# SonghuaHu-UMD/MultiSTGraph

Hardware: AMD Instinct MI355X
Metric: forward node-steps/s (B*T*N per second), MultiATGCN.predict (higher is better)
Workload: dtype f32; 1 GPU; Baltimore 403-node, in=24h out=24h, batch=64/GPU, multi+unidirection K=5; nodes=403, per_gpu_batch=64, global_batch=64, in_steps=24, out_steps=24, parallelism=batch shards, no data-path collective (dp1), layer_wavefront_streams=True

## Files before the change

multistgraph_amd/csrc/matgcn_bwd.hip:

```cpp

namespace {

template <class V, size_t n, class Match, class Args>
int launch_chain(const V (&table)[n], Match match, const dim3& grid, int lds, hipStream_t s, const Args& a) {
  const V* v = find_variant(table, match);
  if (!v) return MATGCN_ERR_UNSUPPORTED;
  hipLaunchKernelGGL(v->fn, grid, dim3(512), lds, s, a);
  CHECK_LAUNCH();
  return MATGCN_OK;
}
constexpr int MAX_FUSED_PARTS = 4;
struct ChainResVariant { bool carry; int parts; bool bf; void (*fn)(ChainResNodeArgs); };
const ChainResVariant CHAIN_RES[] = {
    {false, 0, false, k_chain_res_node<false, true, 0>}, {false, 0, true, k_chain_res_node<false, true, 0, true>},
    {true, 0, false, k_chain_res_node<true, true, 0>},   {true, 0, true, k_chain_res_node<true, true, 0, true>},
    {true, 1, false, k_chain_res_node<true, true, 1>},   {true, 1, true, k_chain_res_node<true, true, 1, true>},
    {true, 2, false, k_chain_res_node<true, true, 2>},   {true, 2, true, k_chain_res_node<true, true, 2, true>},
    {true, 3, false, k_chain_res_node<true, true, 3>},   {true, 3, true, k_chain_res_node<true, true, 3, true>},
    {true, MAX_FUSED_PARTS, false, k_chain_res_node<true, true, MAX_FUSED_PARTS>},
    {true, MAX_FUSED_PARTS, true, k_chain_res_node<true, true, MAX_FUSED_PARTS, true>},
};
struct ChainGateVariant { int parts; bool beta, bf; void (*fn)(ChainNodeArgs); };
const ChainGateVariant CHAIN_GATE[] = {
    {0, false, false, k_chain_gate_node<0, false>}, {0, true, false, k_chain_gate_node<0, true>},
// ... 1286 lines not shown
}

}

extern "C" {

int matgcn_train_bytes(const matgcn_dims* dims, size_t* bytes) {
  if (!bytes) return MATGCN_ERR_NULL;
  Plan P;
  RETURN_IF(make_plan(dims, &P));
  TrainPlan R;
  RETURN_IF(make_train_plan(P, &R));
  *bytes = (size_t)((g_train_precision == 2 && !P.gcnOff ? R.floatsBf16 : R.floats) + (g_deterministic ? R.detFloats : 0)) *
           sizeof(float);
  return MATGCN_OK;
}

static int forward_train_impl(const matgcn_dims* dims, const matgcn_params* params, const void* prepared, const float* X,
                              const matgcn_series* src, const float* h0, const float* drop_mask, float* out,
                              void* workspace, size_t workspace_bytes, void* train, size_t train_bytes, void* stream) {
  if (!prepared || (!X && !src) || !out || !train) return MATGCN_ERR_NULL;
  if (src) RETURN_IF(check_series(dims, src->series, src->series_steps, src->label_start, src->rel_steps));
  Ctx c;
  RETURN_IF(make_ctx(&c, dims, params, prepared, workspace, workspace_bytes, stream, false));
  if (!params->weight_tsg || !params->end_conv_bias) return MATGCN_ERR_NULL;
  for (int h = 0; h < dims->n_heads; ++h) if (!params->weight_ts[h]) return MATGCN_ERR_NULL;
  RETURN_IF(check_layer_params(dims, params));
  const Plan& P = c.P;
  RETURN_IF(make_train_plan(P, &c.R));
  if (train_bytes < (size_t)c.R.floats * sizeof(float)) return MATGCN_ERR_SMALL_BUFFER;
  c.train = (float*)train;
  const int mode = g_train_precision;
  if (mode == 2 && !P.gcnOff && (workspace_bytes < (size_t)P.workspaceFloatsBf16 * sizeof(float) ||
                                 train_bytes < (size_t)c.R.floatsBf16 * sizeof(float)))
    return MATGCN_ERR_SMALL_BUFFER;
  c.prec = precision_of(mode);
  note_train_mode(train, -1);
  if (P.Np != P.N) {
    const size_t rows = (size_t)(c.R.savedFloats / ((long)P.Np * H));
    hipLaunchKernelGGL(k_zero_pad_rows, dim3(blocks_for(rows * (P.Np - P.N) * H)), dim3(256), 0, c.s, c.train,
                       (int)rows, P.N, P.Np, H);
    CHECK_LAUNCH();
  }
  RETURN_IF(wavefront_ready());
  const bool side = g_wavefront_mode != 0;
  hipStream_t aux = side ? g_wf.aux : c.s;
  if (side) {
    HIP_OK(hipEventRecord(g_wf.auxFork, c.s));
    HIP_OK(hipStreamWaitEvent(aux, g_wf.auxFork, 0));
  }
  RETURN_IF(plain_operands(c, c.train, aux, mode == 2 && !P.gcnOff));
  if (side) HIP_OK(hipEventRecord(g_wf.auxDone, aux));
  float* x0p = c.ws + P.oX0p;
  if (src) RETURN_IF(fuse_padded(c, src->series, x0p, src->label_start, src->rel_steps, src->series_steps));
  else RETURN_IF(fuse_padded(c, X, x0p));
  const bool fusedDrop = drop_mask != nullptr && !P.gcnOff;
  if (fusedDrop) c.dropMask = drop_mask;
  RETURN_IF(encoder_padded(c, x0p, h0, nullptr));
  if (side) HIP_OK(hipStreamWaitEvent(c.s, g_wf.auxDone, 0));
  const float* seqTop = c.ws + P.oSeq[P.L - 1];
  if (fusedDrop) {
    seqTop = c.train + c.R.oSeqDrop;
  } else if (drop_mask) {
    const size_t ofs = (size_t)(P.T - P.headT) * P.B * P.Np * H;
    float* dropped = c.train + c.R.oSeqDrop;
    hipLaunchKernelGGL(k_apply_mask, dim3(blocks_for((size_t)P.headT * P.B * P.Np * H)), dim3(256), 0, c.s, seqTop + ofs,
                       drop_mask, dropped + ofs, P.B, P.headT, P.N, P.Np);
    CHECK_LAUNCH();
    seqTop = dropped;
  }
  RETURN_IF(head_padded(c, seqTop, out));
  note_train_mode(train, mode);
  return MATGCN_OK;
}

static int forward_train_entry(const matgcn_dims* dims, const matgcn_params* params, const void* prepared, const float* X,
                               const matgcn_series* src, const float* h0, const float* drop_mask, float* out, void* workspace,
                               size_t workspace_bytes, void* train, size_t train_bytes, void* stream) {
  JOINED(forward_train_impl(dims, params, prepared, X, src, h0, drop_mask, out, workspace, workspace_bytes, train,
                            train_bytes, stream), stream);
}

int matgcn_forward_train(const matgcn_dims* dims, const matgcn_params* params, const void* prepared, const float* X,
                         const matgcn_series* src, const float* h0, const float* drop_mask, float* out, void* workspace,
                         size_t workspace_bytes, void* train, size_t train_bytes, void* stream) {
  return on_main_stream(stream, [&](void* s) {
    return forward_train_entry(dims, params, prepared, X, src, h0, drop_mask, out, workspace, workspace_bytes, train,
                               train_bytes, s);
  });
}

static int backward_entry(const matgcn_dims* dims, const matgcn_params* params, const void* prepared, const float* X,
                          const matgcn_series* src, const float* h0, const float* drop_mask, const float* d_out,
                          const matgcn_grads* grads, float* d_h0, void* workspace, size_t workspace_bytes, void* train,
                          size_t train_bytes, void* stream) {
  if (!prepared || (!X && !src) || !d_out || !grads || !train) return MATGCN_ERR_NULL;
  if (src) RETURN_IF(check_series(dims, src->series, src->series_steps, src->label_start, src->rel_steps));
  Bwd b;
  RETURN_IF(make_ctx(&b.c, dims, params, prepared, workspace, workspace_bytes, stream));
  RETURN_IF(check_layer_params(dims, params));
  RETURN_IF(make_train_plan(b.c.P, &b.c.R));
  if (train_bytes < (size_t)b.c.R.floats * sizeof(float)) return MATGCN_ERR_SMALL_BUFFER;
  b.X = X; b.dropMask = drop_mask; b.g = grads; b.tr = (float*)train;
  b.hasH0 = h0 != nullptr; b.dH0 = d_h0; b.src = src;
  const int mode = train_mode_of(train);
  if (mode < 0) return MATGCN_ERR_BAD_ARG;
  if (mode == 2 && !b.c.P.gcnOff && train_bytes < (size_t)b.c.R.floatsBf16 * sizeof(float)) return MATGCN_ERR_SMALL_BUFFER;
  b.c.prec = precision_of(mode);
  if (g_deterministic) {
    const long base = mode == 2 && !b.c.P.gcnOff ? b.c.R.floatsBf16 : b.c.R.floats;
    if (train_bytes < (size_t)(base + b.c.R.detFloats) * sizeof(float)) return MATGCN_ERR_SMALL_BUFFER;
// ... 34 lines not shown
```

multistgraph_amd/csrc/matgcn_capi.hip:

```cpp
#include <hip/hip_runtime.h>
#include <stdint.h>
#include <stdio.h>
#include <stdlib.h>
#include <string.h>

#include "../../include/matgcn.h"
#include "matgcn_internal.h"

#include "matgcn_kernels.hip"
#include "matgcn_node16.hip"
#include "matgcn_bwd_kernels.hip"

namespace {

constexpr int H = 64;
constexpr int MAX_STEPS = 64;
constexpr int X_CHUNK = 2;

inline long rup(long v, long m) { return (v + m - 1) / m * m; }

struct Plan {
  int B, N, Np, T, L, C0, Ks, Ktot, nFirst, Mp, Kx, d, CH, NTc, od, Tc;
  int per, KtotOrig, nDenseFirst;
  int sumDense;
// ... 580 lines not shown
  const dim3 grid((unsigned)(a.nRowTiles * ((a.nColTiles * 64 + tile.cols - 1) / tile.cols)), (unsigned)a.parts);
  hipLaunchKernelGGL(v->fn, grid, dim3(256), 0, s, a);
  return launch_ok();
}

inline bool mix_flush(MixPrec prec, const MixArgs& a) { return prec != MIX_BF16 && a.nK > 64; }
inline bool mix_half_tiles(MixPrec prec, const MixArgs& a) {
  return prec == MIX_F32 && !mix_flush(prec, a) && a.nColTiles <= 16 && a.xTileStride % 4 == 0 && a.ldX >= 64;
}
inline bool mix_x3_ok(const MixArgs& a) { return a.Apl != nullptr && a.xTileStride % 2 == 0 && a.ldX % 2 == 0; }

struct MixOps { MixPrec prec; const float* St; const void* planes; };
inline MixOps mix_ops(const Ctx& c) {
  return MixOps{c.prec.mix, c.prep + c.P.oSt, c.prec.mix == MIX_BF16X3 ? c.ws + c.P.oPlanes : nullptr};
}

int launch_mix(const Plan& P, const MixOps& m, const float* X, long xTileStride, int ldX, int nColTiles,
               float* out, long sN, long sK, long sT, int Ks, int rowsM, hipStream_t s, bool stepRole = false,
               long outFloats = 0) {
  if (Ks <= 0 || rowsM <= 0) return MATGCN_OK;
  MixArgs a;
  a.St = m.St; a.ldS = P.Mp; a.X = X; a.xTileStride = xTileStride; a.ldX = ldX;
  a.Apl = m.planes; a.plStride = P.planeWords;
  a.out = out; a.sN = sN; a.sK = sK; a.sT = sT; a.outFloats = outFloats;
  a.Np = P.Np; a.N = P.N; a.Ks = Ks; a.nK = P.Np / 16; a.nColTiles = nColTiles;
  ProfScope prof(stepRole ? MATGCN_PROF_MIX : MATGCN_PROF_MIX_PRE, s);
  const MixPrec prec = m.prec;
  if (prec == MIX_BF16X3 && !mix_x3_ok(a)) return MATGCN_ERR_UNSUPPORTED;
  const MixTile tile = prec == MIX_BF16X3 ? MIX_64x128 : mix_half_tiles(prec, a) ? MIX_64x32 : MIX_64x64;
  return launch_mix_variant(tile, prec, mix_flush(prec, a), stepRole ? 1 : 0, a, rowsM, s);
}

int mix_rows(const Plan& P, const MixOps& m, const float* X, int rows, float* G, hipStream_t s, bool stepRole = false,
             long nodeStride = 0) {
  const long sN = nodeStride ? nodeStride : (long)rows * P.Ks * H;
  return launch_mix(P, m, X, (long)P.Np * H, H, rows, G, sN, H, (long)P.Ks * H, P.Ks, P.Ks * P.Np, s, stepRole,
                    (long)(P.N - 1) * sN + (long)rows * P.Ks * H);
}

int lds_opt_in(const void* kernel, int bytes) {
  HIP_OK(hipFuncSetAttribute(kernel, hipFuncAttributeMaxDynamicSharedMemorySize, bytes));
  return MATGCN_OK;
}
int node_kernels_ready(int ldsBytes) {
  int& ready = dev_current().nodeLds;
  if (ready >= ldsBytes) return MATGCN_OK;
  for (const NodeVariant& v : GATE16) RETURN_IF(lds_opt_in(reinterpret_cast<const void*>(v.fn), v.lds));
  for (const NodeVariant& v : UPDATE16) RETURN_IF(lds_opt_in(reinterpret_cast<const void*>(v.fn), v.lds));
  for (const PxVariant& v : PX16) RETURN_IF(lds_opt_in(reinterpret_cast<const void*>(v.fn), ldsBytes));
  ready = ldsBytes;
  return MATGCN_OK;
}

int fold_x0(const Ctx& c, const float* xin, int Tq, hipStream_t s) {
  const Plan& P = c.P;
  const int rows = P.B * Tq;
  const int ld = (int)rup((long)rows * P.C0, 64);
  float* X0m = c.ws + P.oX0m;
  float* MX0 = c.ws + P.oMX0;
  hipLaunchKernelGGL(k_x0_to_matrix, dim3(blocks_for((size_t)P.Np * ld)), dim3(256), 0, s, xin, X0m, rows, P.Np, P.C0,
                     ld);
  CHECK_LAUNCH();
  RETURN_IF(launch_mix(P, mix_ops(c), X0m, 64, ld, ld / 64, MX0, (long)ld, (long)P.Np * ld, 64, P.Ks, P.Ks * P.Np, s));
  hipLaunchKernelGGL(k_build_xa0, dim3(blocks_for((size_t)Tq * P.N * P.B * P.Kx)), dim3(256), 0, s, xin, MX0,
                     c.ws + P.oXA0, P.B, Tq, P.N, P.Np, P.C0, P.Ks, P.Kx, ld);
  return launch_ok();
}

inline int chunk_steps(const Plan& P, int t) {
  int nt = (t < 2) ? 1 : (t < 4 ? 2 : P.Tc);
  if (nt > P.Tc) nt = P.Tc;
  if (t + nt > P.T) nt = P.T - t;
  return nt;
}

int hoist_x(const Ctx& c, int l, const float* xin, int t0, int nt, hipStream_t s, int mixedSteps = 0) {
  const Plan& P = c.P;
  const int rows = P.B * nt;
  float* GX = (c.train ? c.train + c.R.oGX[l] : c.ws + P.oGX[l]) + (size_t)t0 * P.N * P.B * P.Ks * H;
  if (mixedSteps < nt) {
    const int r0 = mixedSteps * P.B;
    RETURN_IF(mix_rows(P, mix_ops(c), xin + (size_t)mixedSteps * P.B * P.Np * H, rows - r0,
                       GX + (size_t)r0 * P.Ks * H, s, false, mixedSteps ? (long)rows * P.Ks * H : 0));
  }
  Px16Args a;
  a.x = xin; a.g = GX; a.w = c.prep + P.oWx[l]; a.bias = c.prep + P.oBx[l];
  a.pxOut = c.ws + P.oPX[l] + (size_t)t0 * P.N * P.RB * NODE_PX_BLOCK;
  a.steps = nt; a.N = P.N; a.Np = P.Np; a.Ks = P.Ks; a.B = P.B;
  ProfScope prof(MATGCN_PROF_PX, s);
  const dim3 grid((unsigned)(rup(P.N, 8) * nt * P.RB));
  const bool bf = c.prec.node;
  if (bf) a.w = c.ws + P.oW16x[l];
  const int nrt = P.B <= 16 ? 1 : P.B <= 32 ? 2 : 4;
  const PxVariant* v = find_variant(PX16, [&](auto& e) { return e.nrt == nrt && e.bf == bf; });
  if (!v) return MATGCN_ERR_UNSUPPORTED;
  hipLaunchKernelGGL(v->fn, grid, dim3(512), P.nodeLds, s, a);
  return launch_ok();
}

bool shared_mix_slot(const Ctx& c, int l, int t, float** g, long* nodeStride) {
  const Plan& P = c.P;
  if (P.gcnOff || l + 1 >= P.L || t < 0 || t >= P.T || P.Ks <= 0) return false;
  int t0 = 0;
  while (t0 + chunk_steps(P, t0) <= t) t0 += chunk_steps(P, t0);
  const int nt = chunk_steps(P, t0);
  const size_t gStep = (size_t)P.N * P.B * P.Ks * H;
  *g = (c.train ? c.train + c.R.oGX[l + 1] : c.ws + P.oGX[l + 1]) + t0 * gStep + (size_t)(t - t0) * P.B * P.Ks * H;
  *nodeStride = (long)nt * P.B * P.Ks * H;
  return true;
}

void fill_res_args(const Ctx& c, int l, const float* xt, long xRowStride, const float* blend, float* seq_t,
                   Node16Args* a) {
  const Plan& P = c.P;
  a->xt = xt; a->xRowStride = xRowStride; a->C = P.Cl[l]; a->Cpad = P.Cpad[l];
// ... 24 lines not shown
  else a.px = c.ws + P.oPX[l] + (size_t)t * P.N * P.RB * NODE_PX_BLOCK;
  const bool save = c.train != nullptr && res != nullptr;
  const bool rows32 = (P.B <= 32 || P.N <= 256) && res != nullptr && !raw && !c.prec.node;
  const dim3 grid(node_items(P.N, P.B, rows32 ? 32 : 64));
  if (save) {
    const size_t at = (size_t)t * P.B * P.Np * H;
    a.svZ = c.train + c.R.oZ[l] + at; a.svR = c.train + c.R.oR[l] + at; a.svHC = c.train + c.R.oHC[l] + at;
    a.svZ2 = c.train + c.R.oZ2[l] + at; a.svR2 = c.train + c.R.oR2[l] + at; a.svHC2 = c.train + c.R.oHC2[l] + at;
  }
  const bool bf = c.prec.node && res != nullptr && !raw;
  if (phase == 1) {
    a.s = Hx; a.w = bf ? c.ws + P.oW16g[l] : c.prep + P.oWg[l]; a.zh = ZHx; a.r = R; a.raw = raw;
    ProfScope prof(MATGCN_PROF_GATE, s);
    return launch_node(GATE16, 0, save, rows32 ? 32 : 64, bf, zeroState, grid, s, a);
  }
  a.s = ZHx; a.w = bf ? c.ws + P.oW16u[l] : c.prep + P.oWu[l]; a.r = R; a.h = Hx; a.hout = Hx;
  ProfScope prof(MATGCN_PROF_UPDATE, s);
  if (res) {
    a.xt = res->xt; a.xRowStride = res->xRowStride; a.C = res->C; a.Cpad = res->Cpad;
    a.rg = res->rg; a.rgb = res->rgb; a.ru = res->ru; a.rub = res->rub;
    a.blend = res->blend; a.seq = res->seq; a.seqRowStride = res->seqRowStride;
    if (save && c.dropMask && l == P.L - 1 && t >= P.T - P.headT && a.seq) {
      a.dropMask = c.dropMask + (size_t)(t - (P.T - P.headT)) * P.N * H;
      a.dropRowStride = (long)P.headT * P.N * H;
      a.seqDrop = c.train + c.R.oSeqDrop + (a.seq - (c.ws + P.oSeq[l]));
    }
  }
  return launch_node(UPDATE16, res ? 1 : 0, save, rows32 ? 32 : 64, bf, zeroState, grid, s, a);
}

int cell_step(const Ctx& c, int l, int t, float* raw, bool gateOnly, const Node16Args* res, hipStream_t s) {
  RETURN_IF(cell_phase(c, l, t, 0, raw, res, s));
  RETURN_IF(cell_phase(c, l, t, 1, raw, res, s));
  if (gateOnly) return MATGCN_OK;
  RETURN_IF(cell_phase(c, l, t, 2, nullptr, res, s));
  return cell_phase(c, l, t, 3, nullptr, res, s);
}

int res_step(const Ctx& c, int l, const float* xt, long xRowStride) {
  const Plan& P = c.P;
  Node16Args a;
  memset(&a, 0, sizeof(a));
  a.s = c.ws + P.oHx[l]; a.hout = c.ws + P.oHx[l];
  a.rows = P.B; a.N = P.N; a.Np = P.Np; a.Ks = P.Ks;
  fill_res_args(c, l, xt, xRowStride, nullptr, nullptr, &a);
  ProfScope prof(MATGCN_PROF_RES, c.s);
  return launch_node(UPDATE16, 2, false, 64, false, false, dim3(node_items(P.N, P.B, 64)), c.s, a);
}

int zero_async(float* p, long floats, hipStream_t s) {
  return hipMemsetAsync(p, 0, (size_t)floats * sizeof(float), s) == hipSuccess ? MATGCN_OK : MATGCN_ERR_LAUNCH;
}

int encoder_chains(const Ctx& c, const float* x0p, const float* h0User, float* finalsUser) {
  const Plan& P = c.P;
  RETURN_IF(node_kernels_ready(P.nodeLds));
  RETURN_IF(wavefront_ready());
  Wavefront& W = g_wf;
  const bool multi = P.L > 1 && g_wavefront_mode != 0;
  const bool lazyPrep = prep_current().pending;
  const bool zeroStart = !h0User && !c.train && !P.gcnOff;
  if (lazyPrep && (!multi || c.prec.node || P.gcnOff)) RETURN_IF(prep_wait(c.s, 3));
  if (c.prec.node && !P.gcnOff) {
    if (c.wsBytes < (size_t)P.workspaceFloatsBf16 * sizeof(float)) return MATGCN_ERR_SMALL_BUFFER;
    for (int l = 0; l < P.L; ++l) {
      const size_t og = (size_t)(P.wgFloats[l] / 8), ou = (size_t)(P.wuFloats[l] / 8);
      hipLaunchKernelGGL(k_stream_to_bf16, dim3(blocks_for(og)), dim3(256), 0, c.s, c.prep + P.oWg[l],
                         reinterpret_cast<unsigned int*>(c.ws + P.oW16g[l]), og);
      CHECK_LAUNCH();
      hipLaunchKernelGGL(k_stream_to_bf16, dim3(blocks_for(ou)), dim3(256), 0, c.s, c.prep + P.oWu[l],
                         reinterpret_cast<unsigned int*>(c.ws + P.oW16u[l]), ou);
      CHECK_LAUNCH();
      if (l > 0) {
        const size_t ox = (size_t)((long)P.N * P.wxStride / 8);
        hipLaunchKernelGGL(k_stream_to_bf16, dim3(blocks_for(ox)), dim3(256), 0, c.s, c.prep + P.oWx[l],
                           reinterpret_cast<unsigned int*>(c.ws + P.oW16x[l]), ox);
        CHECK_LAUNCH();
      }
    }
  }
  if (c.prec.mix == MIX_BF16X3 && P.Ks > 0) {
    if (c.wsBytes < (size_t)P.workspaceFloatsX3 * sizeof(float)) return MATGCN_ERR_SMALL_BUFFER;
    hipLaunchKernelGGL(k_split_bf16x3, dim3(blocks_for((size_t)P.planeWords)), dim3(256), 0, c.s, c.prep + P.oSt, P.Mp, P.Np,
                       P.nKg, reinterpret_cast<uint4*>(c.ws + P.oPlanes), P.planeWords);
    CHECK_LAUNCH();
  }
  if (multi) {
    HIP_OK(hipEventRecord(W.fork, c.s));
    for (int l = 1; l < P.L; ++l) {
      HIP_OK(hipStreamWaitEvent(W.chain[l], W.fork, 0));
      HIP_OK(hipStreamWaitEvent(W.xpart[l], W.fork, 0));
      if (lazyPrep) {
        RETURN_IF(prep_wait(W.chain[l], 2));
        RETURN_IF(prep_wait(W.xpart[l], 2));
      }
    }
  }
  if (!P.gcnOff) RETURN_IF(fold_x0(c, x0p, P.T, c.s));
  const long stepRows = (long)P.B * P.Np * H;
  auto chain_stream = [&](int l) { return (l == 0 || !multi) ? c.s : W.chain[l]; };
  for (int l = 0; l < P.L; ++l) {
    hipStream_t cs = chain_stream(l);
    RETURN_IF(zero_async(c.ws + P.oZHx[l], (long)P.B * P.Np * H, cs));
    if (P.Np != P.N) {
      hipLaunchKernelGGL(k_zero_pad_rows, dim3(blocks_for((size_t)P.B * P.T * (P.Np - P.N) * H)), dim3(256), 0, cs,
                         c.ws + P.oSeq[l], P.B * P.T, P.N, P.Np, H);
      CHECK_LAUNCH();
    }
    hipLaunchKernelGGL(k_pack_rows, dim3(blocks_for((size_t)P.B * P.Np * H)), dim3(256), 0, cs,
                       h0User ? h0User + (size_t)l * P.B * P.N * H : nullptr,
                       c.ws + P.oHx[l], P.B, P.N, P.Np, H);
    CHECK_LAUNCH();
    if (c.train && h0User) {
      hipLaunchKernelGGL(k_pack_rows, dim3(blocks_for((size_t)P.B * P.Np * H)), dim3(256), 0, cs,
                         h0User + (size_t)l * P.B * P.N * H, c.train + c.R.oH0 + (size_t)l * P.B * P.Np * H, P.B, P.N,
                         P.Np, H);
      CHECK_LAUNCH();
    }
  }
  int nextChunk[MATGCN_MAX_LAYERS] = {0};
  auto enqueue_step = [&](int l, int t) -> int {
    hipStream_t cs = chain_stream(l);
    hipStream_t xs = multi ? W.xpart[l] : c.s;
    const float* below = (l == 0) ? nullptr : c.ws + P.oSeq[l - 1];
    float* seq = c.ws + P.oSeq[l];
    if (P.gcnOff) {
      if (multi && l > 0) HIP_OK(hipStreamWaitEvent(cs, W.step[l - 1][t], 0));
      Node16Args a;
      memset(&a, 0, sizeof(a));
      a.s = c.ws + P.oHx[l]; a.hout = c.ws + P.oHx[l];
      a.rows = P.B; a.N = P.N; a.Np = P.Np; a.Ks = 0;
      if (l == 0) fill_res_args(c, l, x0p + (long)t * P.Np * P.C0, (long)P.T * P.Np * P.C0, nullptr, seq + t * stepRows, &a);
      else fill_res_args(c, l, below + t * stepRows, (long)P.Np * H, nullptr, seq + t * stepRows, &a);
      {
        ProfScope prof(MATGCN_PROF_RES, cs);
        if (c.train) {
          const size_t at = (size_t)t * P.B * P.Np * H;
          a.svZ2 = c.train + c.R.oZ2[l] + at; a.svR2 = c.train + c.R.oR2[l] + at; a.svHC2 = c.train + c.R.oHC2[l] + at;
        }
        RETURN_IF(launch_node(UPDATE16, 2, c.train != nullptr, 64, false, false, dim3(node_items(P.N, P.B, 64)), cs, a));
      }
      CHECK_LAUNCH();
      if (multi && l + 1 < P.L) HIP_OK(hipEventRecord(W.step[l][t], cs));
      return MATGCN_OK;
    }
    if (l > 0 && t == nextChunk[l]) {
      const int nt = chunk_steps(P, t);
      nextChunk[l] = t + nt;
      float* slot; long stride;
      int mixedSteps = 0;
      if (shared_mix_slot(c, l - 1, t, &slot, &stride)) mixedSteps = P.T - 1 - t < nt ? P.T - 1 - t : nt;
      if (multi) {
        if (mixedSteps == nt) HIP_OK(hipStreamWaitEvent(xs, W.mixed[l - 1][t + nt], 0));
        else HIP_OK(hipStreamWaitEvent(xs, W.step[l - 1][t + nt - 1], 0));
      }
      RETURN_IF(hoist_x(c, l, below + t * stepRows, t, nt, xs, mixedSteps));
      if (multi) {
        HIP_OK(hipEventRecord(W.xdone[l][t], xs));
        HIP_OK(hipStreamWaitEvent(cs, W.xdone[l][t], 0));
      }
    }
    Node16Args res;
    if (l == 0)
      fill_res_args(c, l, x0p + (long)t * P.Np * P.C0, (long)P.T * P.Np * P.C0,
                    c.prm->weights_gru + (size_t)l * P.T + t, seq + t * stepRows, &res);
    else
      fill_res_args(c, l, below + t * stepRows, (long)P.Np * H, c.prm->weights_gru + (size_t)l * P.T + t,
                    seq + t * stepRows, &res);
    const bool zs = zeroStart && t == 0;
    if (!zs) RETURN_IF(cell_phase(c, l, t, 0, nullptr, &res, cs));
    if (multi && l + 1 < P.L) HIP_OK(hipEventRecord(W.mixed[l][t], cs));
    if (lazyPrep && multi && l == 0 && t == 0) RETURN_IF(prep_wait(cs, 1));
    RETURN_IF(cell_phase(c, l, t, 1, nullptr, &res, cs, zs));
    if (!zs) RETURN_IF(cell_phase(c, l, t, 2, nullptr, &res, cs));
    RETURN_IF(cell_phase(c, l, t, 3, nullptr, &res, cs, zs));
    if (multi && l + 1 < P.L) HIP_OK(hipEventRecord(W.step[l][t], cs));
    return MATGCN_OK;
  };
  for (int l = 0; l < P.L; ++l)
    for (int t = 0; t < P.T; ++t) RETURN_IF(enqueue_step(l, t));
  for (int l = 0; l < P.L; ++l) {
    hipStream_t cs = chain_stream(l);
    if (finalsUser) {
      hipLaunchKernelGGL(k_unpack_rows, dim3(blocks_for((size_t)P.B * P.N * H)), dim3(256), 0, cs, c.ws + P.oHx[l],
                         finalsUser + (size_t)l * P.B * P.N * H, P.B, P.N, P.Np, H);
      CHECK_LAUNCH();
    }
    if (multi && l > 0) HIP_OK(hipEventRecord(W.done[l], cs));
  }
  if (multi)
    for (int l = 1; l < P.L; ++l) HIP_OK(hipStreamWaitEvent(c.s, W.done[l], 0));
  return MATGCN_OK;
}

int encoder_padded(const Ctx& c, const float* x0p, const float* h0User, float* finalsUser) {
  const int rc = encoder_chains(c, x0p, h0User, finalsUser);
  if (rc != MATGCN_OK) join_library_streams(c.s);
  return rc;
}

int fuse_padded(const Ctx& c, const float* X, float* x0p, const int32_t* labelStart = nullptr,
                const int32_t* relSteps = nullptr, int64_t seriesSteps = 0) {
  const Plan& P = c.P;
  const matgcn_dims* D = c.D;
  RETURN_IF(zero_async(x0p, (long)P.B * P.T * P.Np * P.C0, c.s));
  FuseArgs a;
  memset(&a, 0, sizeof(a));
  a.X = X; a.x0 = x0p; a.tsg = c.prm->weight_tsg;
  a.labelStart = labelStart; a.seriesSteps = (long)seriesSteps;
  if (labelStart)
    for (int s2 = 0; s2 < D->x_steps; ++s2) a.rel[s2] = relSteps[s2];
  for (int h = 0; h < D->n_heads; ++h) { a.ts[h] = c.prm->weight_ts[h]; a.headBegin[h] = D->head_begin[h]; }
  for (int j = 0; j < P.C0 - P.od; ++j) a.extSrc[j] = D->ext_src[j];
  a.B = P.B; a.T = P.T; a.N = P.N; a.Np = P.Np; a.C0 = P.C0; a.od = P.od; a.F = D->x_feat;
  a.xSteps = D->x_steps; a.startDim = D->start_dim; a.nHeads = D->n_heads; a.nTs = D->n_ts;
  hipLaunchKernelGGL(k_fuse_heads, dim3(blocks_for((size_t)P.B * P.T * P.N)), dim3(256), 0, c.s, a);
  return launch_ok();
}

int head_padded(const Ctx& c, const float* seqp, float* out) {
  const Plan& P = c.P;
  HeadArgs a;
  a.seq = seqp + (size_t)(P.T - P.headT) * P.B * P.Np * H; a.w = c.prep + P.oHead;
  a.bias = c.prm->end_conv_bias; a.out = out;
  a.B = P.B; a.T = P.headT; a.N = P.N; a.Np = P.Np; a.CH = P.CH; a.od = P.od; a.NTc = P.NTc;
  ProfScope prof(MATGCN_PROF_HEAD, c.s);
  hipLaunchKernelGGL(k_head, dim3((unsigned)(P.B * ((P.N + 31) / 32))), dim3(256), 0, c.s, a);
  return launch_ok();
}

int make_ctx(Ctx* c, const matgcn_dims* dims, const matgcn_params* params, const void* prepared, void* workspace,
             size_t workspace_bytes, void* stream, bool joinPrepare = true) {
  if (!dims || !params || !workspace) return MATGCN_ERR_NULL;
  RETURN_IF(make_plan(dims, &c->P));
  if (workspace_bytes < (size_t)c->P.workspaceFloats * sizeof(float)) return MATGCN_ERR_SMALL_BUFFER;
  c->D = dims; c->prm = params; c->prep = (const float*)prepared; c->ws = (float*)workspace;
  c->wsBytes = workspace_bytes;
  c->s = (hipStream_t)stream;
  if (prepared && joinPrepare) RETURN_IF(prep_wait(c->s, 3));
  return MATGCN_OK;
}

int check_layer_params(const matgcn_dims* D, const matgcn_params* p) {
  if (!D->gcn_off && (!p->node_emb || !p->weights_gru)) return MATGCN_ERR_NULL;
  for (int l = 0; l < D->layers; ++l) {
    if (!p->res_gate[l].weight || !p->res_gate[l].bias || !p->res_update[l].weight || !p->res_update[l].bias)
      return MATGCN_ERR_NULL;
    if (D->gcn_off) continue;
    if (!p->gate[l].weights_pool || !p->gate[l].bias_pool || !p->update[l].weights_pool || !p->update[l].bias_pool)
      return MATGCN_ERR_NULL;
    if (D->scale_by_g && (!p->gate[l].weights_g || !p->update[l].weights_g)) return MATGCN_ERR_NULL;
    if (!p->res_gate[l].weight || !p->res_gate[l].bias || !p->res_update[l].weight || !p->res_update[l].bias)
      return MATGCN_ERR_NULL;
  }
  return MATGCN_OK;
}

int stage_single_step(const Ctx& c, int layer, const float* x, const float* h, bool xpart, float** xin_out) {
  const Plan& P = c.P;
  if (layer < 0 || layer >= P.L) return MATGCN_ERR_BAD_ARG;
  if (P.gcnOff && xpart) return MATGCN_ERR_UNSUPPORTED;
  RETURN_IF(node_kernels_ready(P.nodeLds));
  float* xin = (layer == 0) ? c.ws + P.oX0p : c.ws + P.oSeq[layer - 1];
  hipLaunchKernelGGL(k_pack_rows, dim3(blocks_for((size_t)P.B * P.Np * P.Cl[layer])), dim3(256), 0, c.s, x, xin, P.B,
                     P.N, P.Np, P.Cl[layer]);
  CHECK_LAUNCH();
  hipLaunchKernelGGL(k_pack_rows, dim3(blocks_for((size_t)P.B * P.Np * H)), dim3(256), 0, c.s, h, c.ws + P.oHx[layer],
                     P.B, P.N, P.Np, H);
  CHECK_LAUNCH();
// ... 297 lines not shown
      if (l == 0) {
        if (!fast) {
          q.baseOfs = (long)nG * 16 * O; q.kind = 1; q.iOfs = 0; q.groups = P.nGx[0];
          hipLaunchKernelGGL(k_prep_stream<1>, dim3(blocks_for((size_t)q.groups * (O / 16) * 64), nodeGroups), dim3(256), 0,
                             ws, q);
          CHECK_LAUNCH();
        }
      } else {
        q.out = prep + P.oWx[l]; q.nodeStride = P.wxStride; q.baseOfs = 0;
        q.kind = 0; q.iOfs = 0; q.groups = nG; q.OTdst = 12; q.otOfs = part == 0 ? 0 : 8;
        if (fast)
          launch_fast(q, O, ws);
        else
          hipLaunchKernelGGL(k_prep_stream<0>, dim3(blocks_for((size_t)q.groups * (O / 16) * 64), nodeGroups), dim3(256), 0,
                             ws, q);
        CHECK_LAUNCH();
        hipLaunchKernelGGL(k_prep_bias, dim3(blocks_for((size_t)P.N * O)), dim3(256), 0, ws, params->node_emb,
                           ap.bias_pool, P.d, O, P.N, prep + P.oBx[l], 192, part == 0 ? 0 : 128);
        CHECK_LAUNCH();
      }
    }
    if (lazy && l == 0) {
      HIP_OK(hipEventRecord(E.l0[0], pool[1]));
      HIP_OK(hipEventRecord(E.l0[1], pool[2]));
    }
    const int nG1 = (P.Cpad[l] + H) / 16;
    hipLaunchKernelGGL(k_prep_linear16, dim3(blocks_for((size_t)nG1 * 8 * 64)), dim3(256), 0, c.s,
                       params->res_gate[l].weight, I, 128, P.Cl[l], P.Cpad[l], nG1, prep + P.oRg[l]);
    CHECK_LAUNCH();
    hipLaunchKernelGGL(k_prep_linear16, dim3(blocks_for((size_t)nG1 * 4 * 64)), dim3(256), 0, c.s,
                       params->res_update[l].weight, I, 64, P.Cl[l], P.Cpad[l], nG1, prep + P.oRu[l]);
    CHECK_LAUNCH();
  }
  hipLaunchKernelGGL(k_prep_linear, dim3(blocks_for((size_t)(P.headT * H / 8) * P.NTc * 64)), dim3(256), 0, c.s,
                     params->end_conv_weight, P.headT * H, P.CH, 0, 0, P.headT * H, P.NTc, prep + P.oHead);
  CHECK_LAUNCH();
  if (lazy) {
    HIP_OK(hipEventRecord(E.l1[0], pool[1]));
    HIP_OK(hipEventRecord(E.l1[1], pool[2]));
    E.pending = true;
  } else if (fork) {
    HIP_OK(hipEventRecord(W.done[1], pool[1]));
    HIP_OK(hipEventRecord(W.done[2], pool[2]));
    HIP_OK(hipStreamWaitEvent(c.s, W.done[1], 0));
    HIP_OK(hipStreamWaitEvent(c.s, W.done[2], 0));
  }
  return MATGCN_OK;
}

static int forward_once(Ctx& c, const float* X, const float* series, int64_t seriesSteps, const int32_t* labelStart,
                        const int32_t* relSteps, const float* h0, float* out) {
  const Plan& P = c.P;
  float* x0p = c.ws + P.oX0p;
  if (series) RETURN_IF(fuse_padded(c, series, x0p, labelStart, relSteps, seriesSteps));
  else RETURN_IF(fuse_padded(c, X, x0p));
  RETURN_IF(encoder_padded(c, x0p, h0, nullptr));
  return head_padded(c, c.ws + P.oSeq[P.L - 1], out);
}

static int forward_entry(const matgcn_dims* dims, const matgcn_params* params, const void* prepared, const float* X,
                         const float* h0, float* out, void* workspace, size_t workspace_bytes, void* stream) {
  if (!prepared || !X || !out) return MATGCN_ERR_NULL;
  Ctx c;
  RETURN_IF(make_ctx(&c, dims, params, prepared, workspace, workspace_bytes, stream, false));
  if (!params->weight_tsg || !params->end_conv_bias) return MATGCN_ERR_NULL;
  for (int h = 0; h < dims->n_heads; ++h) if (!params->weight_ts[h]) return MATGCN_ERR_NULL;
  RETURN_IF(check_layer_params(dims, params));
  c.prec = precision_of(g_mix_precision);
  return forward_once(c, X, nullptr, 0, nullptr, nullptr, h0, out);
}

int matgcn_forward(const matgcn_dims* dims, const matgcn_params* params, const void* prepared, const float* X,
                   const float* h0, float* out, void* workspace, size_t workspace_bytes, void* stream) {
  return on_main_stream(stream, [&](void* s) {
    return forward_entry(dims, params, prepared, X, h0, out, workspace, workspace_bytes, s);
  });
}

static int check_series(const matgcn_dims* dims, const float* series, int64_t series_steps, const int32_t* label_start,
                 const int32_t* rel_steps) {
  if (!series || !label_start || !rel_steps) return MATGCN_ERR_NULL;
  if (dims->x_steps > MATGCN_MAX_XSTEPS) return MATGCN_ERR_UNSUPPORTED;
  int lo = 0;
  for (int s2 = 0; s2 < dims->x_steps; ++s2) lo = rel_steps[s2] < lo ? rel_steps[s2] : lo;
  if (series_steps < 1 || -(int64_t)lo >= series_steps) return MATGCN_ERR_BAD_ARG;
  return MATGCN_OK;
}

static int forward_series_entry(const matgcn_dims* dims, const matgcn_params* params, const void* prepared,
                                const float* series, int64_t series_steps, const int32_t* label_start,
                                const int32_t* rel_steps, const float* h0, float* out, void* workspace,
                                size_t workspace_bytes, void* stream) {
  if (!prepared || !series || !label_start || !rel_steps || !out) return MATGCN_ERR_NULL;
  Ctx c;
  RETURN_IF(make_ctx(&c, dims, params, prepared, workspace, workspace_bytes, stream, false));
  if (!params->weight_tsg || !params->end_conv_bias) return MATGCN_ERR_NULL;
  for (int h = 0; h < dims->n_heads; ++h) if (!params->weight_ts[h]) return MATGCN_ERR_NULL;
  RETURN_IF(check_layer_params(dims, params));
  RETURN_IF(check_series(dims, series, series_steps, label_start, rel_steps));
  c.prec = precision_of(g_mix_precision);
  return forward_once(c, nullptr, series, series_steps, label_start, rel_steps, h0, out);
}

int matgcn_forward_series(const matgcn_dims* dims, const matgcn_params* params, const void* prepared,
                          const float* series, int64_t series_steps, const int32_t* label_start,
                          const int32_t* rel_steps, const float* h0, float* out, void* workspace,
                          size_t workspace_bytes, void* stream) {
  return on_main_stream(stream, [&](void* s) {
    return forward_series_entry(dims, params, prepared, series, series_steps, label_start, rel_steps, h0, out, workspace,
                                workspace_bytes, s);
  });
}

int matgcn_fuse_heads(const matgcn_dims* dims, const matgcn_params* params, const float* X, float* x0,
                      void* workspace, size_t workspace_bytes, void* stream) {
  if (!X || !x0) return MATGCN_ERR_NULL;
  Ctx c;
  RETURN_IF(make_ctx(&c, dims, params, nullptr, workspace, workspace_bytes, stream));
  if (!params->weight_tsg) return MATGCN_ERR_NULL;
  for (int h = 0; h < dims->n_heads; ++h) if (!params->weight_ts[h]) return MATGCN_ERR_NULL;
  const Plan& P = c.P;
  float* x0p = c.ws + P.oX0p;
  RETURN_IF(fuse_padded(c, X, x0p));
  hipLaunchKernelGGL(k_unpack_rows, dim3(blocks_for((size_t)P.B * P.T * P.N * P.C0)), dim3(256), 0, c.s, x0p, x0,
                     P.B * P.T, P.N, P.Np, P.C0);
  return launch_ok();
}

int matgcn_agcn_gate_fwd(const matgcn_dims* dims, const matgcn_params* params, const void* prepared, int layer,
                         const float* x, const float* h, float* y, void* workspace, size_t workspace_bytes,
                         void* stream) {
  if (!prepared || !x || !h || !y) return MATGCN_ERR_NULL;
  Ctx c;
  RETURN_IF(make_ctx(&c, dims, params, prepared, workspace, workspace_bytes, stream));
  float* xin;
  RETURN_IF(stage_single_step(c, layer, x, h, true, &xin));
  return cell_step(c, layer, 0, y, true, nullptr, c.s);
}

int matgcn_atgru_cell_fwd(const matgcn_dims* dims, const matgcn_params* params, const void* prepared, int layer,
                          const float* x, const float* h, float* h_out, void* workspace, size_t workspace_bytes,
                          void* stream) {
  if (!prepared || !x || !h || !h_out) return MATGCN_ERR_NULL;
  Ctx c;
  RETURN_IF(make_ctx(&c, dims, params, prepared, workspace, workspace_bytes, stream));
  const Plan& P = c.P;
  float* xin;
  RETURN_IF(stage_single_step(c, layer, x, h, true, &xin));
  RETURN_IF(cell_step(c, layer, 0, nullptr, false, nullptr, c.s));
  hipLaunchKernelGGL(k_unpack_rows, dim3(blocks_for((size_t)P.B * P.N * H)), dim3(256), 0, c.s, c.ws + P.oHx[layer],
                     h_out, P.B, P.N, P.Np, H);
  return launch_ok();
}

int matgcn_res_cell_fwd(const matgcn_dims* dims, const matgcn_params* params, const void* prepared, int layer,
                        const float* x, const float* h, float* h_out, void* workspace, size_t workspace_bytes,
                        void* stream) {
  if (!prepared || !x || !h || !h_out) return MATGCN_ERR_NULL;
  Ctx c;
  RETURN_IF(make_ctx(&c, dims, params, prepared, workspace, workspace_bytes, stream));
  const Plan& P = c.P;
  float* xin;
  RETURN_IF(stage_single_step(c, layer, x, h, false, &xin));
  RETURN_IF(res_step(c, layer, xin, (long)P.Np * P.Cl[layer]));
  hipLaunchKernelGGL(k_unpack_rows, dim3(blocks_for((size_t)P.B * P.N * H)), dim3(256), 0, c.s, c.ws + P.oHx[layer],
                     h_out, P.B, P.N, P.Np, H);
  return launch_ok();
}

int matgcn_encoder_fwd(const matgcn_dims* dims, const matgcn_params* params, const void* prepared, const float* x0,
                       const float* h0, float* seq, float* finals, void* workspace, size_t workspace_bytes,
                       void* stream) {
  if (!prepared || !x0) return MATGCN_ERR_NULL;
  Ctx c;
  RETURN_IF(make_ctx(&c, dims, params, prepared, workspace, workspace_bytes, stream));
  RETURN_IF(check_layer_params(dims, params));
// ... 67 lines not shown
```

multistgraph_amd/csrc/matgcn_internal.h:

```cpp
#ifndef MATGCN_INTERNAL_H
#define MATGCN_INTERNAL_H
#include <stddef.h>
#include <stdint.h>

#define MATGCN_MAX_STACK 16

struct StackMap {
  int KtotOrig;
  int nKeep;
  int keepK[MATGCN_MAX_STACK];
  int nDiag;
  int diagK[MATGCN_MAX_STACK];
  int diagOrder[MATGCN_MAX_STACK];
  const float* diagSrc[MATGCN_MAX_STACK];
  int N;
};

struct StackEntries {
  int n;
  int pool[2 * MATGCN_MAX_STACK];
  int slot[2 * MATGCN_MAX_STACK];
  int diag[2 * MATGCN_MAX_STACK];
};

struct PrepStream {
  const float* E;
  const float* wpool;
  const float* bpool;
  const float* wg;
  float* out;
  long nodeStride;
  long baseOfs;
  int d, I, O, N;
  int kind;
  int iOfs, C0;
  int groups;
  int groupsX;
  int OTdst, otOfs;
  StackMap map;
};

struct FuseArgs {
  const float* X;
  const int* labelStart;
  int rel[256];
  long seriesSteps;
  float* x0;
  const float* tsg;
  const float* ts[8];
  int B, T, N, Np, C0, od, F, xSteps, startDim, nHeads, nTs;
  int headBegin[8];
  int extSrc[16];
};

struct MixArgs {
  const float* St = nullptr;
  int ldS = 0;
  const float* X = nullptr;
  long xTileStride = 0;
  int ldX = 0;
  float* out = nullptr;
  long sN = 0, sK = 0, sT = 0;
  long outFloats = 0;
  int Np = 0, N = 0, Ks = 0, nK = 0, nColTiles = 0, nRowTiles = 0;
  int parts = 1;
  long aPartStride = 0, xPartStride = 0, outPartStride = 0;
  const void* Apl = nullptr;
  long plStride = 0;
};

struct HeadArgs {
  const float* seq;
  const float* w;
  const float* bias;
  float* out;
  int B, T, N, Np, CH, od, NTc;
};

#endif
```

multistgraph_amd/csrc/matgcn_kernels.hip:

```cpp
#include <hip/hip_runtime.h>
#include <stdint.h>

#include "matgcn_internal.h"

typedef __attribute__((ext_vector_type(16))) float f32x16;
typedef unsigned int u32x4 __attribute__((ext_vector_type(4)));
typedef __attribute__((ext_vector_type(4))) float f32x4;
#define MFMA16(a, b, c) __builtin_amdgcn_mfma_f32_16x16x4f32((a), (b), (c), 0, 0, 0)

#define MFMA32(a, b, c) __builtin_amdgcn_mfma_f32_32x32x2f32((a), (b), (c), 0, 0, 0)

__device__ __forceinline__ float sigmoid_f(float x) { return 1.0f / (1.0f + expf(-x)); }

__device__ __forceinline__ int acc_row(int r, int half) { return (r & 3) + 8 * (r >> 2) + 4 * half; }

__global__ __launch_bounds__(256) void k_adaptive_adj(const float* __restrict__ e1, const float* __restrict__ e2,
                                                      int rank, int bidir, int N, float* __restrict__ plain, int ldP) {
  extern __shared__ float logits[];
  __shared__ float red[256];
  __shared__ float erow[64];
  const int n = blockIdx.x, tid = threadIdx.x;
  for (int r = tid; r < rank; r += 256) erow[r] = e1[(size_t)n * rank + r];
  __syncthreads();
  float mx = 0.f;
// ... 362 lines not shown
                                                     int N, int Np, int C) {
  const size_t idx = (size_t)blockIdx.x * 256 + threadIdx.x;
  const size_t total = (size_t)rows * N * C;
  if (idx >= total) return;
  const int c = idx % C;
  const int n = (idx / C) % N;
  const size_t r = idx / ((size_t)C * N);
  dst[idx] = src[(r * Np + n) * C + c];
}

__global__ __launch_bounds__(256) void k_pack_seq_tm(const float* __restrict__ src, float* __restrict__ dst, int B,
                                                     int T, int N, int Np, int C) {
  const size_t idx = (size_t)blockIdx.x * 256 + threadIdx.x;
  const size_t total = (size_t)T * B * Np * C;
  if (idx >= total) return;
  const int c = idx % C;
  const int n = (idx / C) % Np;
  const int b = (idx / ((size_t)C * Np)) % B;
  const int t = idx / ((size_t)C * Np * B);
  dst[idx] = (n < N) ? src[(((size_t)b * T + t) * N + n) * C + c] : 0.f;
}

__global__ __launch_bounds__(256) void k_unpack_seq_tm(const float* __restrict__ src, float* __restrict__ dst, int B,
                                                       int T, int N, int Np, int C) {
  const size_t idx = (size_t)blockIdx.x * 256 + threadIdx.x;
  const size_t total = (size_t)B * T * N * C;
  if (idx >= total) return;
  const int c = idx % C;
  const int n = (idx / C) % N;
  const int t = (idx / ((size_t)C * N)) % T;
  const int b = idx / ((size_t)C * N * T);
  dst[idx] = src[(((size_t)t * B + b) * Np + n) * C + c];
}

__global__ __launch_bounds__(256) void k_zero_pad_rows(float* __restrict__ buf, int rows, int N, int Np, int C) {
  const int per = (Np - N) * C;
  const size_t idx = (size_t)blockIdx.x * 256 + threadIdx.x;
  if (idx >= (size_t)rows * per) return;
  const size_t r = idx / per;
  const int q = idx - r * per;
  buf[(r * Np + N) * C + q] = 0.f;
}

struct PadRowBufs { float* p[8]; };
__global__ __launch_bounds__(256) void k_zero_pad_rows_multi(PadRowBufs bufs, int rows, int N, int Np, int C) {
  const int per4 = (Np - N) * C / 4;
  const size_t idx = (size_t)blockIdx.x * 256 + threadIdx.x;
  if (idx >= (size_t)rows * per4) return;
  const size_t r = idx / per4;
  const int q = (int)(idx - r * per4);
  *reinterpret_cast<float4*>(bufs.p[blockIdx.y] + (r * Np + N) * C + 4 * q) = make_float4(0.f, 0.f, 0.f, 0.f);
}

__device__ unsigned long long g_series_violations = 0;
__device__ __forceinline__ size_t series_row(long row, long steps) {
  if (row < 0 || row >= steps) {
    atomicAdd(&g_series_violations, 1ull);
    row = row < 0 ? 0 : steps - 1;
  }
  return (size_t)row;
}

__global__ __launch_bounds__(256) void k_fuse_heads(FuseArgs a) {
  const size_t idx = (size_t)blockIdx.x * 256 + threadIdx.x;
  const size_t total = (size_t)a.B * a.T * a.N;
  if (idx >= total) return;
  const int n = idx % a.N;
  const int t = (idx / a.N) % a.T;
  const int b = idx / ((size_t)a.N * a.T);
  float gmax = -3.0e38f, gsum = 0.f;
  for (int h = 0; h < a.nTs; ++h) gmax = fmaxf(gmax, a.tsg[h]);
  for (int h = 0; h < a.nTs; ++h) gsum += expf(a.tsg[h] - gmax);
  auto xrow = [&](int step) -> const float* {
    const size_t r = a.labelStart ? series_row((long)a.labelStart[b] + a.rel[step], a.seriesSteps)
                                  : (size_t)b * a.xSteps + step;
    return a.X + (r * a.N + n) * a.F;
  };
  float* dst = a.x0 + (((size_t)b * a.T + t) * a.Np + n) * a.C0;
  for (int c = 0; c < a.od; ++c) {
    float acc = 0.f;
    for (int h = 0; h < a.nHeads; ++h) {
      const float g = expf(a.tsg[h] - gmax) / gsum;
      const float xv = xrow(a.headBegin[h] + t)[a.startDim + c];
      const float wv = a.ts[h][((size_t)t * a.N + n) * a.od + c];
      acc += g * xv * wv;
    }
    dst[c] = acc;
  }
  for (int j = 0; j < a.C0 - a.od; ++j)
    dst[a.od + j] = xrow(t)[a.extSrc[j]];
}

__global__ __launch_bounds__(256) void k_x0_to_matrix(const float* __restrict__ x0p, float* __restrict__ X0m, int rows,
                                                      int Np, int C0, int ld) {
  const size_t idx = (size_t)blockIdx.x * 256 + threadIdx.x;
  const size_t total = (size_t)Np * ld;
  if (idx >= total) return;
  const int col = idx % ld;
  const int m = idx / ld;
  float v = 0.f;
  if (col < rows * C0) {
    const int row = col / C0, c = col - row * C0;
    v = x0p[((size_t)row * Np + m) * C0 + c];
  }
  X0m[idx] = v;
}

__global__ __launch_bounds__(256) void k_build_xa0(const float* __restrict__ x0p, const float* __restrict__ MX0,
                                                   float* __restrict__ XA0, int B, int T, int N, int Np, int C0,
                                                   int Ks, int Kx, int ld) {
  const size_t idx = (size_t)blockIdx.x * 256 + threadIdx.x;
  const size_t total = (size_t)T * N * B * Kx;
  if (idx >= total) return;
  const int j = idx % Kx;
  const int b = (idx / Kx) % B;
  const int n = (idx / ((size_t)Kx * B)) % N;
  const int t = idx / ((size_t)Kx * B * N);
  const int row = b * T + t;
  float v = 0.f;
  const int nx = (Ks + 1) * C0;
  if (j < C0) v = x0p[((size_t)row * Np + n) * C0 + j];
  else if (j < nx) {
    const int k = j / C0 - 1, c = j % C0;
    v = MX0[((size_t)k * Np + n) * ld + (size_t)row * C0 + c];
  } else if (j == nx) v = 1.0f;
  XA0[idx] = v;
}

constexpr int MIX_FLUSH_TILES = 16;

__device__ __forceinline__ void mix_tile_order(int id, int nColUnits, int nRowTiles, int& rowTile, int& colUnit) {
  if ((nColUnits & 7) == 0) {
    const int xcd = id & 7, j = id >> 3, cpx = nColUnits >> 3;
    rowTile = j % nRowTiles;
    colUnit = xcd * cpx + j / nRowTiles;
  } else {
    rowTile = id % nRowTiles;
    colUnit = id / nRowTiles;
  }
}

template <int ROLE, bool FLUSH = false>
__global__ __launch_bounds__(256) void k_mix(MixArgs a) {
// ... 889 lines not shown
```

Before: 94.76 million node-steps/s.

## Fuse x0 matrix transpose into head-fusion kernel and merge encoder init launches

```diff
diff --git a/multistgraph_amd/csrc/matgcn_bwd.hip b/multistgraph_amd/csrc/matgcn_bwd.hip
--- a/multistgraph_amd/csrc/matgcn_bwd.hip
+++ b/multistgraph_amd/csrc/matgcn_bwd.hip
@@ -1362,11 +1362,11 @@
   RETURN_IF(plain_operands(c, c.train, aux, mode == 2 && !P.gcnOff));
   if (side) HIP_OK(hipEventRecord(g_wf.auxDone, aux));
   float* x0p = c.ws + P.oX0p;
-  if (src) RETURN_IF(fuse_padded(c, src->series, x0p, src->label_start, src->rel_steps, src->series_steps));
-  else RETURN_IF(fuse_padded(c, X, x0p));
+  if (src) RETURN_IF(fuse_padded(c, src->series, x0p, !P.gcnOff, src->label_start, src->rel_steps, src->series_steps));
+  else RETURN_IF(fuse_padded(c, X, x0p, !P.gcnOff));
   const bool fusedDrop = drop_mask != nullptr && !P.gcnOff;
   if (fusedDrop) c.dropMask = drop_mask;
-  RETURN_IF(encoder_padded(c, x0p, h0, nullptr));
+  RETURN_IF(encoder_padded(c, x0p, h0, nullptr, !P.gcnOff));
   if (side) HIP_OK(hipStreamWaitEvent(c.s, g_wf.auxDone, 0));
   const float* seqTop = c.ws + P.oSeq[P.L - 1];
   if (fusedDrop) {
diff --git a/multistgraph_amd/csrc/matgcn_capi.hip b/multistgraph_amd/csrc/matgcn_capi.hip
--- a/multistgraph_amd/csrc/matgcn_capi.hip
+++ b/multistgraph_amd/csrc/matgcn_capi.hip
@@ -656,15 +656,17 @@
   return MATGCN_OK;
 }
 
-int fold_x0(const Ctx& c, const float* xin, int Tq, hipStream_t s) {
+int fold_x0(const Ctx& c, const float* xin, int Tq, hipStream_t s, bool haveMatrix = false) {
   const Plan& P = c.P;
   const int rows = P.B * Tq;
   const int ld = (int)rup((long)rows * P.C0, 64);
   float* X0m = c.ws + P.oX0m;
   float* MX0 = c.ws + P.oMX0;
-  hipLaunchKernelGGL(k_x0_to_matrix, dim3(blocks_for((size_t)P.Np * ld)), dim3(256), 0, s, xin, X0m, rows, P.Np, P.C0,
-                     ld);
-  CHECK_LAUNCH();
+  if (!haveMatrix) {
+    hipLaunchKernelGGL(k_x0_to_matrix, dim3(blocks_for((size_t)P.Np * ld)), dim3(256), 0, s, xin, X0m, rows, P.Np, P.C0,
+                       ld);
+    CHECK_LAUNCH();
+  }
   RETURN_IF(launch_mix(P, mix_ops(c), X0m, 64, ld, ld / 64, MX0, (long)ld, (long)P.Np * ld, 64, P.Ks, P.Ks * P.Np, s));
   hipLaunchKernelGGL(k_build_xa0, dim3(blocks_for((size_t)Tq * P.N * P.B * P.Kx)), dim3(256), 0, s, xin, MX0,
                      c.ws + P.oXA0, P.B, Tq, P.N, P.Np, P.C0, P.Ks, P.Kx, ld);
@@ -795,10 +797,22 @@
   return hipMemsetAsync(p, 0, (size_t)floats * sizeof(float), s) == hipSuccess ? MATGCN_OK : MATGCN_ERR_LAUNCH;
 }
 
-int encoder_chains(const Ctx& c, const float* x0p, const float* h0User, float* finalsUser) {
+int encoder_chains(const Ctx& c, const float* x0p, const float* h0User, float* finalsUser, bool x0Matrix) {
   const Plan& P = c.P;
   RETURN_IF(node_kernels_ready(P.nodeLds));
   RETURN_IF(wavefront_ready());
+  {
+    InitArgs ia;
+    memset(&ia, 0, sizeof(ia));
+    for (int l = 0; l < P.L; ++l) {
+      ia.zhx[l] = c.ws + P.oZHx[l]; ia.hx[l] = c.ws + P.oHx[l]; ia.seq[l] = c.ws + P.oSeq[l];
+      if (c.train && h0User) ia.h0copy[l] = c.train + c.R.oH0 + (size_t)l * P.B * P.Np * H;
+    }
+    ia.h0 = h0User; ia.B = P.B; ia.N = P.N; ia.Np = P.Np; ia.seqRows = P.B * P.T;
+    const size_t units = ((size_t)P.B * P.Np + (size_t)P.B * P.T * (P.Np - P.N)) * (H / 4);
+    hipLaunchKernelGGL(k_forward_init, dim3(blocks_for(units), (unsigned)P.L), dim3(256), 0, c.s, ia);
+    CHECK_LAUNCH();
+  }
   Wavefront& W = g_wf;
   const bool multi = P.L > 1 && g_wavefront_mode != 0;
   const bool lazyPrep = prep_current().pending;
@@ -839,28 +853,9 @@
       }
     }
   }
-  if (!P.gcnOff) RETURN_IF(fold_x0(c, x0p, P.T, c.s));
+  if (!P.gcnOff) RETURN_IF(fold_x0(c, x0p, P.T, c.s, x0Matrix));
   const long stepRows = (long)P.B * P.Np * H;
   auto chain_stream = [&](int l) { return (l == 0 || !multi) ? c.s : W.chain[l]; };
-  for (int l = 0; l < P.L; ++l) {
-    hipStream_t cs = chain_stream(l);
-    RETURN_IF(zero_async(c.ws + P.oZHx[l], (long)P.B * P.Np * H, cs));
-    if (P.Np != P.N) {
-      hipLaunchKernelGGL(k_zero_pad_rows, dim3(blocks_for((size_t)P.B * P.T * (P.Np - P.N) * H)), dim3(256), 0, cs,
-                         c.ws + P.oSeq[l], P.B * P.T, P.N, P.Np, H);
-      CHECK_LAUNCH();
-    }
-    hipLaunchKernelGGL(k_pack_rows, dim3(blocks_for((size_t)P.B * P.Np * H)), dim3(256), 0, cs,
-                       h0User ? h0User + (size_t)l * P.B * P.N * H : nullptr,
-                       c.ws + P.oHx[l], P.B, P.N, P.Np, H);
-    CHECK_LAUNCH();
-    if (c.train && h0User) {
-      hipLaunchKernelGGL(k_pack_rows, dim3(blocks_for((size_t)P.B * P.Np * H)), dim3(256), 0, cs,
-                         h0User + (size_t)l * P.B * P.N * H, c.train + c.R.oH0 + (size_t)l * P.B * P.Np * H, P.B, P.N,
-                         P.Np, H);
-      CHECK_LAUNCH();
-    }
-  }
   int nextChunk[MATGCN_MAX_LAYERS] = {0};
   auto enqueue_step = [&](int l, int t) -> int {
     hipStream_t cs = chain_stream(l);
@@ -936,20 +931,20 @@
   return MATGCN_OK;
 }
 
-int encoder_padded(const Ctx& c, const float* x0p, const float* h0User, float* finalsUser) {
-  const int rc = encoder_chains(c, x0p, h0User, finalsUser);
+int encoder_padded(const Ctx& c, const float* x0p, const float* h0User, float* finalsUser, bool x0Matrix = false) {
+  const int rc = encoder_chains(c, x0p, h0User, finalsUser, x0Matrix);
   if (rc != MATGCN_OK) join_library_streams(c.s);
   return rc;
 }
 
-int fuse_padded(const Ctx& c, const float* X, float* x0p, const int32_t* labelStart = nullptr,
+int fuse_padded(const Ctx& c, const float* X, float* x0p, bool x0Matrix, const int32_t* labelStart = nullptr,
                 const int32_t* relSteps = nullptr, int64_t seriesSteps = 0) {
   const Plan& P = c.P;
   const matgcn_dims* D = c.D;
-  RETURN_IF(zero_async(x0p, (long)P.B * P.T * P.Np * P.C0, c.s));
   FuseArgs a;
   memset(&a, 0, sizeof(a));
   a.X = X; a.x0 = x0p; a.tsg = c.prm->weight_tsg;
+  if (x0Matrix) { a.x0m = c.ws + P.oX0m; a.ld = P.nc0p; }
   a.labelStart = labelStart; a.seriesSteps = (long)seriesSteps;
   if (labelStart)
     for (int s2 = 0; s2 < D->x_steps; ++s2) a.rel[s2] = relSteps[s2];
@@ -957,7 +952,9 @@
   for (int j = 0; j < P.C0 - P.od; ++j) a.extSrc[j] = D->ext_src[j];
   a.B = P.B; a.T = P.T; a.N = P.N; a.Np = P.Np; a.C0 = P.C0; a.od = P.od; a.F = D->x_feat;
   a.xSteps = D->x_steps; a.startDim = D->start_dim; a.nHeads = D->n_heads; a.nTs = D->n_ts;
-  hipLaunchKernelGGL(k_fuse_heads, dim3(blocks_for((size_t)P.B * P.T * P.N)), dim3(256), 0, c.s, a);
+  const long tileRows = x0Matrix ? (P.nc0p + P.C0 - 1) / P.C0 : (long)P.B * P.T;
+  const dim3 grid((unsigned)((P.Np / 16) * ((tileRows + 15) / 16)));
+  hipLaunchKernelGGL(k_fuse_heads, grid, dim3(256), 256 * P.C0 * sizeof(float), c.s, a);
   return launch_ok();
 }
 
@@ -1361,9 +1358,9 @@
                         const int32_t* relSteps, const float* h0, float* out) {
   const Plan& P = c.P;
   float* x0p = c.ws + P.oX0p;
-  if (series) RETURN_IF(fuse_padded(c, series, x0p, labelStart, relSteps, seriesSteps));
-  else RETURN_IF(fuse_padded(c, X, x0p));
-  RETURN_IF(encoder_padded(c, x0p, h0, nullptr));
+  if (series) RETURN_IF(fuse_padded(c, series, x0p, !P.gcnOff, labelStart, relSteps, seriesSteps));
+  else RETURN_IF(fuse_padded(c, X, x0p, !P.gcnOff));
+  RETURN_IF(encoder_padded(c, x0p, h0, nullptr, !P.gcnOff));
   return head_padded(c, c.ws + P.oSeq[P.L - 1], out);
 }
 
@@ -1430,7 +1427,7 @@
   for (int h = 0; h < dims->n_heads; ++h) if (!params->weight_ts[h]) return MATGCN_ERR_NULL;
   const Plan& P = c.P;
   float* x0p = c.ws + P.oX0p;
-  RETURN_IF(fuse_padded(c, X, x0p));
+  RETURN_IF(fuse_padded(c, X, x0p, false));
   hipLaunchKernelGGL(k_unpack_rows, dim3(blocks_for((size_t)P.B * P.T * P.N * P.C0)), dim3(256), 0, c.s, x0p, x0,
                      P.B * P.T, P.N, P.Np, P.C0);
   return launch_ok();
diff --git a/multistgraph_amd/csrc/matgcn_internal.h b/multistgraph_amd/csrc/matgcn_internal.h
--- a/multistgraph_amd/csrc/matgcn_internal.h
+++ b/multistgraph_amd/csrc/matgcn_internal.h
@@ -46,6 +46,8 @@
   int rel[256];
   long seriesSteps;
   float* x0;
+  float* x0m;
+  int ld;
   const float* tsg;
   const float* ts[8];
   int B, T, N, Np, C0, od, F, xSteps, startDim, nHeads, nTs;
diff --git a/multistgraph_amd/csrc/matgcn_kernels.hip b/multistgraph_amd/csrc/matgcn_kernels.hip
--- a/multistgraph_amd/csrc/matgcn_kernels.hip
+++ b/multistgraph_amd/csrc/matgcn_kernels.hip
@@ -438,6 +438,41 @@
   *reinterpret_cast<float4*>(bufs.p[blockIdx.y] + (r * Np + N) * C + 4 * q) = make_float4(0.f, 0.f, 0.f, 0.f);
 }
 
+struct InitArgs {
+  float* zhx[MATGCN_MAX_LAYERS];
+  float* hx[MATGCN_MAX_LAYERS];
+  float* seq[MATGCN_MAX_LAYERS];
+  float* h0copy[MATGCN_MAX_LAYERS];
+  const float* h0;
+  int B, N, Np, seqRows;
+};
+__global__ __launch_bounds__(256) void k_forward_init(InitArgs a) {
+  const int l = blockIdx.y;
+  const size_t state4 = (size_t)a.B * a.Np * 16;
+  const size_t pad4 = (size_t)a.seqRows * (a.Np - a.N) * 16;
+  size_t idx = (size_t)blockIdx.x * 256 + threadIdx.x;
+  const float4 zero = make_float4(0.f, 0.f, 0.f, 0.f);
+  if (idx < state4) {
+    reinterpret_cast<float4*>(a.zhx[l])[idx] = zero;
+    float4 v = zero;
+    const int n = (int)((idx / 16) % a.Np);
+    if (a.h0 && n < a.N) {
+      const size_t b = idx / ((size_t)16 * a.Np);
+      const float* src = a.h0 + (((size_t)l * a.B + b) * a.N + n) * 64 + 4 * (idx % 16);
+      v = make_float4(src[0], src[1], src[2], src[3]);
+    }
+    reinterpret_cast<float4*>(a.hx[l])[idx] = v;
+    if (a.h0copy[l]) reinterpret_cast<float4*>(a.h0copy[l])[idx] = v;
+    return;
+  }
+  idx -= state4;
+  if (idx >= pad4) return;
+  const size_t per4 = (size_t)(a.Np - a.N) * 16;
+  const size_t r = idx / per4;
+  const size_t q = idx - r * per4;
+  reinterpret_cast<float4*>(a.seq[l] + (r * a.Np + a.N) * 64)[q] = zero;
+}
+
 __device__ unsigned long long g_series_violations = 0;
 __device__ __forceinline__ size_t series_row(long row, long steps) {
   if (row < 0 || row >= steps) {
@@ -448,33 +483,57 @@
 }
 
 __global__ __launch_bounds__(256) void k_fuse_heads(FuseArgs a) {
-  const size_t idx = (size_t)blockIdx.x * 256 + threadIdx.x;
-  const size_t total = (size_t)a.B * a.T * a.N;
-  if (idx >= total) return;
-  const int n = idx % a.N;
-  const int t = (idx / a.N) % a.T;
-  const int b = idx / ((size_t)a.N * a.T);
-  float gmax = -3.0e38f, gsum = 0.f;
-  for (int h = 0; h < a.nTs; ++h) gmax = fmaxf(gmax, a.tsg[h]);
-  for (int h = 0; h < a.nTs; ++h) gsum += expf(a.tsg[h] - gmax);
-  auto xrow = [&](int step) -> const float* {
-    const size_t r = a.labelStart ? series_row((long)a.labelStart[b] + a.rel[step], a.seriesSteps)
-                                  : (size_t)b * a.xSteps + step;
-    return a.X + (r * a.N + n) * a.F;
-  };
-  float* dst = a.x0 + (((size_t)b * a.T + t) * a.Np + n) * a.C0;
-  for (int c = 0; c < a.od; ++c) {
-    float acc = 0.f;
-    for (int h = 0; h < a.nHeads; ++h) {
-      const float g = expf(a.tsg[h] - gmax) / gsum;
-      const float xv = xrow(a.headBegin[h] + t)[a.startDim + c];
-      const float wv = a.ts[h][((size_t)t * a.N + n) * a.od + c];
-      acc += g * xv * wv;
-    }
-    dst[c] = acc;
-  }
-  for (int j = 0; j < a.C0 - a.od; ++j)
-    dst[a.od + j] = xrow(t)[a.extSrc[j]];
+  extern __shared__ float fuseTile[];
+  const int nTilesN = a.Np / 16;
+  const int n0 = (blockIdx.x % nTilesN) * 16;
+  const size_t r0 = (size_t)(blockIdx.x / nTilesN) * 16;
+  const int n = n0 + (threadIdx.x & 15);
+  const size_t row = r0 + (threadIdx.x >> 4);
+  const size_t rows = (size_t)a.B * a.T;
+  float* tile = fuseTile + (size_t)threadIdx.x * a.C0;
+  if (row < rows && n < a.N) {
+    const int t = row % a.T;
+    const int b = row / a.T;
+    float gmax = -3.0e38f, gsum = 0.f;
+    for (int h = 0; h < a.nTs; ++h) gmax = fmaxf(gmax, a.tsg[h]);
+    for (int h = 0; h < a.nTs; ++h) gsum += expf(a.tsg[h] - gmax);
+    auto xrow = [&](int step) -> const float* {
+      const size_t r = a.labelStart ? series_row((long)a.labelStart[b] + a.rel[step], a.seriesSteps)
+                                    : (size_t)b * a.xSteps + step;
+      return a.X + (r * a.N + n) * a.F;
+    };
+    float* dst = a.x0 + (((size_t)b * a.T + t) * a.Np + n) * a.C0;
+    for (int c = 0; c < a.od; ++c) {
+      float acc = 0.f;
+      for (int h = 0; h < a.nHeads; ++h) {
+        const float g = expf(a.tsg[h] - gmax) / gsum;
+        const float xv = xrow(a.headBegin[h] + t)[a.startDim + c];
+        const float wv = a.ts[h][((size_t)t * a.N + n) * a.od + c];
+        acc += g * xv * wv;
+      }
+      dst[c] = acc;
+      tile[c] = acc;
+    }
+    for (int j = 0; j < a.C0 - a.od; ++j) {
+      const float v = xrow(t)[a.extSrc[j]];
+      dst[a.od + j] = v;
+      tile[a.od + j] = v;
+    }
+  } else {
+    if (row < rows) {
+      float* dst = a.x0 + (row * a.Np + n) * a.C0;
+      for (int c = 0; c < a.C0; ++c) dst[c] = 0.f;
+    }
+    for (int c = 0; c < a.C0; ++c) tile[c] = 0.f;
+  }
+  if (!a.x0m) return;
+  __syncthreads();
+  const int w = 16 * a.C0;
+  for (int e = threadIdx.x; e < 16 * w; e += 256) {
+    const int nl = e / w, q = e - nl * w;
+    const size_t col = r0 * a.C0 + q;
+    if (col < (size_t)a.ld) a.x0m[(size_t)(n0 + nl) * a.ld + col] = fuseTile[((q / a.C0) * 16 + nl) * a.C0 + q % a.C0];
+  }
 }
 
 __global__ __launch_bounds__(256) void k_x0_to_matrix(const float* __restrict__ x0p, float* __restrict__ X0m, int rows,
```

After: 94.67 million node-steps/s. No clear change (-0.1%).
